# Kiteretsu77/This_and_That_VDM

Hardware: AMD Instinct MI355X
Metric: denoise-steps/sec (14-frame 256x448 VGL, 25 steps) (higher is better)
Workload: dtype bf16; 1 GPU; VGL denoise step: GestureNet ControlNet + spatio-temporal UNet + per-frame CFG + Euler, latent 14x4x32x56, CFG batch 2, 78 context tokens, heads (5,10,20,20); mode=vgl, requests_per_gpu=1, parallelism=1 independent request(s), one per GPU; RCCL weight broadcast at start-up only, hipgraph=True, finite_output=True, spatial_self_attention=bf16, weights_identical_on_all_ranks=True

## Files before the change

this_and_that_vdm_amd/csrc/gemm.hip:

```cpp
#include <stdlib.h>
#include "gemm_kernel.h"

namespace ttg {
void launch_bf16(GemmP& p, int cfg, hipStream_t st);
void launch_f16(GemmP& p, int cfg, hipStream_t st);
void launch_f32(GemmP& p, int cfg, hipStream_t st);
void launch_sq320_bf16(const GemmP& p, hipStream_t st);
void launch_sq320_f16(const GemmP& p, hipStream_t st);
void launch_pp_bf16(GemmP& p, hipStream_t st);
void launch_pp_f16(GemmP& p, hipStream_t st);
void launch_w320(GemmP& p, hipStream_t st, int bm, bool bf16);
}
using namespace ttg;

namespace {
inline int gemm_taps(int mode) { return mode == 1 || mode == 3 ? 9 : (mode == 2 ? 3 : 1); }

int env_int(const char* name, int dflt) { const char* e = getenv(name); return e ? atoi(e) : dflt; }
int big_tile_bits(int on) { return on == 0 ? 0 : (on == 2 ? 1 : (on == 3 ? 11 : (on == 4 ? 7 : 15))); }
struct Knobs {
  int forced_cfg = env_int("TT_GEMM_CFG", -1);
  int group_m = env_int("TT_GEMM_GROUP_M", 0);
  int forced_split = env_int("TT_GEMM_SPLITK", -1);
  int deep = env_int("TT_GEMM_DEEP", 1);
  int small64 = env_int("TT_GEMM_SMALL64", 2);
  int sq320 = env_int("TT_GEMM_SQ320", 2);
  int sq320_rowvec = env_int("TT_SQ320_ROWVEC", 1);
  int sq320_min_rows = env_int("TT_SQ320_MIN_ROWS", 131072);
  int pp = env_int("TT_GEMM_PP", 1);
  int pp_geglu_min_tiles = env_int("TT_PP_GEGLU_MIN_TILES", 400);
  int pp_geglu_min_fill = env_int("TT_PP_GEGLU_MIN_FILL", 75);
  int pp_min_tiles = env_int("TT_PP_MIN_TILES", 460);
  int pp_min_fill = env_int("TT_PP_MIN_FILL", 90);
  int pp_split_whole = env_int("TT_PP_SPLIT_WHOLE", 1);
  int w320 = big_tile_bits(env_int("TT_GEMM_W320", 1));
  int w320_force = env_int("TT_W320_FORCE", 0);
  int w320_min_fill = env_int("TT_W320_MIN_FILL", 60);
  int f32_split = env_int("TT_F32_SPLIT", 0) ? 1 : 0;
  int f32_split_min_tiles = env_int("TT_F32_SPLIT_MIN_TILES", 160);
// ... 109 lines not shown
    if (head.m < a->m && pp_ok(&head)) return head.m;
  }
  return 0;
}
void pp_split(const TtGemmArgs* a, int rows, TtGemmArgs* head, TtGemmArgs* tail) {
  const size_t es = 2;
  *head = *a; *tail = *a;
  head->m = rows;
  tail->m = a->m - rows;
  tail->a0 = (const char*)a->a0 + (size_t)rows * a->lda0 * es;
  tail->out = (char*)a->out + (size_t)rows * a->ldo * es;
}

const TileCfg& tile_of(int dtype, int cfg) { return dtype == TT_F32 ? kCfgsF32[cfg] : kCfgs[cfg]; }
bool ln_capable(int cfg) { return kCfgs[cfg].ln; }
bool mode3_capable(int cfg) { return kCfgs[cfg].m3; }
Plan mode3_plan(const TtGemmArgs* a, Plan pl) {
  if (a->mode != 3 || a->dtype == TT_F32 || knobs().forced_cfg >= 0 || mode3_capable(pl.cfg)) return pl;
  if (pl.cfg == 20) return Plan{16, pl.splitk};
  const long b128 = (long)ceil_div(a->m, 128) * ceil_div(a->n, 128), b12864 = (long)ceil_div(a->m, 128) * ceil_div(a->n, 64);
  return Plan{b128 >= 384 ? 11 : (b12864 >= 384 ? 1 : 2), 1};
}
bool mode3_served(const TtGemmArgs* a, const Plan& pl) { return a->mode != 3 || tile_of(a->dtype, pl.cfg).m3; }
Plan plan_for(const TtGemmArgs* a) {
  if (a->dtype == TT_F32) {
    const int split_min = knobs().f32_split_min_tiles;
    if (knobs().f32_split) {
      const long b128 = (long)ceil_div(a->m, 128) * ceil_div(a->n, 128);
      const long kt = (long)gemm_taps(a->mode) * (a->k0 + a->k1) / 32;
      if (knobs().f32_splitk && !a->geglu && !a->ln_fold && !a->out_col_hw && b128 < split_min && kt >= 64) {
        long sp = 448 / b128;
        if (sp > kt / 16) sp = kt / 16;
        if (sp > 16) sp = 16;
        if (sp >= 2) return Plan{0, (int)sp};
      }
    }
    return Plan{plan_f32(a->m, a->n, knobs().f32_split ? split_min : 256), 1};
  }
  const long ktot = (long)gemm_taps(a->mode) * (a->k0 + a->k1);
  const bool allow = !a->geglu && !a->ln_fold && !a->out_fp8;
  const bool k128 = (a->k0 & 127) == 0 && (a->k1 & 127) == 0;
  const bool wide_ok = !(a->residual || a->blend || a->rowvec);
  Plan pl = make_plan(knobs().forced_cfg, a->m, a->n, ktot, allow, wide_ok, a->mode == 0, k128);
  if (a->ln_fold && !ln_capable(pl.cfg))
    pl = make_plan(-1, a->m, a->n, ktot, false, wide_ok, a->mode == 0);
  return mode3_plan(a, pl);
}
// ... 14 lines not shown
  if (sq) return Route{Kind::SQ320, -1, 1, 0};
  if (big) return Route{big == 1 ? Kind::W320 : Kind::W320H, -1, 1, 0};
  if (const int split = w320_split(a)) return Route{Kind::W320H_SPLIT, -1, split, 0};
  return tiled_route(a, plan_for(a));
}
Route granted_route(const TtGemmArgs* a, Route r) {
  if (r.kind == Kind::W320H_SPLIT && !ws_fits(a, r.splitk)) r = tiled_route(a, plan_for(a));
  if (r.kind == Kind::TILED && r.splitk > 1 && (!ws_fits(a, r.splitk) || slab_bytes(a, r.splitk) >= ((size_t)1 << 31))) r = tiled_route(a, unsplit_plan(a));
  return r;
}
Route resolve(const TtGemmArgs* a) { return granted_route(a, wanted_route(a)); }

TileCfg route_tile(const TtGemmArgs* a, const Route& r) {
  switch (r.kind) {
    case Kind::PP: case Kind::PP_TWO_PART: return TileCfg{-1, 256, 256, 64, 0, 2, 4};
    case Kind::SQ320: return TileCfg{-1, SQ_ROWS, SQ_N, SQ_K, a->residual ? 3 : 5, 1, SQ_WAVES};
    case Kind::W320: return TileCfg{-1, 256, 320, 64, 0, 4, 2};
    case Kind::W320H: case Kind::W320H_SPLIT: return TileCfg{-1, 128, 320, 64, 0, 2, 2};
    default: return tile_of(a->dtype, r.cfg);
  }
}

int32_t stats_rows_on(const TtGemmArgs* a, const Route& r) {
  if (a->geglu || a->out_fp8 || a->out_f32 || a->out_col_hw > 0 || a->ln_fold == 2) return 0;
  if (r.kind == Kind::PP || r.kind == Kind::PP_TWO_PART || r.kind == Kind::SQ320 || r.kind == Kind::UNSUPPORTED) return 0;
  const int seg = a->stats_seg;
  if (r.splitk != 1) {
    if (seg <= 0) return 0;
    for (int rows = seg < 128 ? seg : 128; rows > 0; --rows)
      if (seg % rows == 0) return a->m % rows == 0 ? rows : 0;
    return 0;
  }
  const TileCfg t = route_tile(a, r);
  if (a->blend && !(a->blend == a->residual && a->ld_blend == a->ld_res)) return 0;
  if (a->rowvec && a->rowvec_rows < 32 && !(a->rowvec_rows == 1 && a->rowvec_mod == 2)) return 0;
  if (t.bm > 128 && t.bn != 320 && a->residual) return 0;
  if (a->dtype == TT_F32 && knobs().f32_split && a->residual) return 0;
  if (t.bn == 320 || t.nst == 0) {
    if (a->m % t.bm) return 0;
    return (t.bm == 128 && seg > 0 && seg % 128 && seg % 64 == 0) ? 64 : t.bm;
  }
  const int wave_rows = t.bm / t.wgm;
  const int rows = (seg <= 0 || seg % t.bm == 0) ? t.bm : (seg % wave_rows == 0 ? wave_rows : t.bm);
  return a->m % rows == 0 ? rows : 0;
}
int32_t gn_fused_on(const TtGemmArgs* a, const Route& r) {
  if (a->dtype == TT_F32 || a->geglu || a->out_fp8 || a->out_f32 || a->out_col_hw > 0 || a->stats_out) return 0;
  const int seg = a->stats_seg;
  if (seg <= 0 || a->m % seg || (a->n & 127)) return 0;
  if (r.kind != Kind::W320H_SPLIT && r.kind != Kind::TILED) return 0;
  if (r.splitk <= 1) return 0;
  return splitk_gn_rows(seg, a->n, nullptr) > 0 ? 1 : 0;
}
}

int tt_internal_f32_split() { return knobs().f32_split; }

extern "C" int tt_gemm_set_tile_override(int32_t cfg) {
  if (cfg < -1 || cfg >= kNumCfgs) TT_FAIL(TT_EINVAL, "tt_gemm_set_tile_override: cfg %d (valid -1..%d)", cfg, kNumCfgs - 1);
  knobs().forced_cfg = cfg;
  return TT_OK;
}
extern "C" int tt_gemm_set_streaming_square(int32_t on) {
  knobs().sq320 = on == 2 ? 2 : (on ? 1 : 0);
  return TT_OK;
}
extern "C" int tt_gemm_set_f32_split(int32_t on) { knobs().f32_split = on ? 1 : 0; return TT_OK; }
extern "C" int tt_gemm_set_big_tile(int32_t on) { knobs().w320 = big_tile_bits(on); return TT_OK; }

extern "C" int tt_gemm_plan(const TtGemmArgs* a, int32_t cfg[7]) {
  if (!a || !cfg || a->m <= 0 || a->n <= 0) TT_FAIL(TT_EINVAL, "tt_gemm_plan: bad arguments");
  const Route r = resolve(a);
  if (r.kind == Kind::UNSUPPORTED)
    TT_FAIL(TT_EUNSUPPORTED, "tt_gemm_plan: forced tile configuration %d has no mode-3 variant (mode 3 is built for 1, 2, 11, 16)", r.cfg);
  const TileCfg t = route_tile(a, r);
  cfg[0] = t.bm; cfg[1] = t.bn; cfg[2] = t.bk; cfg[3] = t.nst; cfg[4] = t.wgm; cfg[5] = t.wgn; cfg[6] = r.splitk;
  return TT_OK;
}

extern "C" int32_t tt_gemm_stats_rows(const TtGemmArgs* a) {
  if (!a || a->m <= 0 || a->n <= 0) return 0;
  return stats_rows_on(a, resolve(a));
}

extern "C" int32_t tt_gemm_gn_fused(const TtGemmArgs* a) {
  if (!a || a->m <= 0 || a->n <= 0) return 0;
  return gn_fused_on(a, resolve(a));
}

extern "C" size_t tt_gemm_ws_bytes(const TtGemmArgs* a) {
  if (!a || a->m <= 0 || a->n <= 0) return 0;
  const Route r = wanted_route(a);
  if (r.kind == Kind::PP_TWO_PART) { TtGemmArgs head, tail; pp_split(a, r.head_rows, &head, &tail); return tt_gemm_ws_bytes(&tail); }
  return (r.kind == Kind::W320H_SPLIT || r.kind == Kind::TILED) && r.splitk > 1 ? slab_bytes(a, r.splitk) : 0;
// ... 28 lines not shown
  p.blend = (const char*)a->blend; p.ld_blend = a->ld_blend; p.alpha = a->alpha;
  const int es = a->dtype == TT_F32 ? 4 : 2;
  p.out = (char*)a->out; p.ldo = a->ldo; p.out_f32 = a->dtype == TT_F32 ? 0 : a->out_f32;
  p.out_col_hw = a->out_col_hw; p.out_col_hwp = a->out_col_hwp;
  p.ln_fold = a->ln_fold; p.ln_eps = a->ln_eps; p.out_fp8 = a->out_fp8; p.stats = a->stats_out; p.stat_rows = a->gn_out ? a->stats_seg : (a->stats_out ? stats_rows_on(a, r) : 0);
  p.f32_split = a->dtype == TT_F32 ? knobs().f32_split : 0;
  p.presplit = a->presplit;
  if (a->presplit) {
    if ((a->presplit & ~3) || a->dtype != TT_F32 || !p.f32_split)
      TT_FAIL(TT_EINVAL, "tt_gemm: presplit operands need TT_F32 with tt_gemm_set_f32_split(1)");
    if (((a->presplit & 1) && a->ln_fold == 1) || ((a->presplit & 2) && a->ln_fold == 2))
      TT_FAIL(TT_EINVAL, "tt_gemm: the LayerNorm statistics cannot be taken from a pre-split operand");
    if ((a->presplit & 1) && a->mode != 0) TT_FAIL(TT_EINVAL, "tt_gemm: a pre-split A operand is a Linear operand (mode 0)");
  }
  p.gn_out = (char*)a->gn_out; p.ld_gn = a->ld_gn; p.gn_gamma = a->gn_gamma; p.gn_beta = a->gn_beta; p.gn_eps = a->gn_eps; p.gn_silu = a->gn_silu;
  if (p.mode == 1 || p.mode == 3) {
    if (p.nimg <= 0 || p.hin <= 0 || p.win <= 0 || p.hout <= 0 || p.wout <= 0 || p.stride < 1)
      TT_FAIL(TT_EINVAL, "tt_gemm: conv geometry");
    if ((long)p.nimg * p.hout * p.wout != p.m) TT_FAIL(TT_EINVAL, "tt_gemm: m != nimg*hout*wout");
  }
  if (p.mode == 2) {
    if (p.frames <= 0 || p.hw <= 0 || p.m % ((long)p.frames * p.hw)) TT_FAIL(TT_EINVAL, "tt_gemm: tconv geometry");
  }
  p.taps = gemm_taps(p.mode);
  {
    const long rows = p.mode == 1 || p.mode == 3 ? (long)p.nimg * p.hin * p.win : (long)p.m;
    const long a0b = ((rows - 1) * p.lda0 + p.k0) * es, a1b = p.k1 ? ((rows - 1) * p.lda1 + p.k1) * es : 16;
    const long wb = ((long)(p.n - 1) * p.ldw + (long)p.taps * (p.k0 + p.k1)) * es;
    if (a0b >= (1L << 31) || a1b >= (1L << 31) || wb >= (1L << 31))
      TT_FAIL(TT_EUNSUPPORTED, "tt_gemm: operand larger than 2 GiB (32-bit buffer offsets)");
    p.a0_bytes = (unsigned)a0b; p.a1_bytes = (unsigned)a1b; p.w_bytes = (unsigned)wb;
    const long n_out = p.geglu ? p.n / 2 : p.n;
    const long outb = ((long)(p.m - 1) * p.ldo + (p.out_col_hw > 0 ? p.ldo : n_out)) * (p.out_f32 ? 4 : (p.out_fp8 ? 1 : es));
    const long resb = p.residual ? ((long)(p.m - 1) * p.ld_res + p.n) * es : 0;
    const long blb = p.blend ? ((long)(p.m - 1) * p.ld_blend + p.n) * es : 0;
    long rv_last = p.rowvec ? (p.m - 1) / p.rowvec_rows : 0;
    if (p.rowvec_mod > 0 && rv_last > p.rowvec_mod - 1) rv_last = p.rowvec_mod - 1;
    const long rvb = p.rowvec ? (rv_last * p.ld_rowvec + p.n) * 4 : 0;
    if (outb >= (1L << 31) || resb >= (1L << 31) || blb >= (1L << 31) || rvb >= (1L << 31))
      TT_FAIL(TT_EUNSUPPORTED, "tt_gemm: epilogue operand larger than 2 GiB (32-bit buffer offsets)");
    p.out_bytes = (unsigned)outb; p.res_bytes = (unsigned)resb; p.blend_bytes = (unsigned)blb;
    p.bias_bytes = p.bias ? (unsigned)p.n * 4u : 0u; p.rowvec_bytes = (unsigned)rvb;
  }
  p.splitk = r.splitk; p.group_m = 1;
  p.group_m_override = r.kind == Kind::PP || r.kind == Kind::TILED ? knobs().group_m : 0;
  p.ws = r.splitk > 1 ? (float*)a->ws : nullptr;
  p.ws_bytes = r.splitk > 1 ? (unsigned)slab_bytes(a, r.splitk) : 0u;
  return TT_OK;
}
}

extern "C" int tt_gemm(const TtGemmArgs* a, tt_stream_t stream) {
  if (!a || !a->a0 || !a->w || !a->out) TT_FAIL(TT_EINVAL, "tt_gemm: null operand");
  if (a->m <= 0 || a->n <= 0 || a->k0 <= 0) TT_FAIL(TT_EINVAL, "tt_gemm: empty problem m=%d n=%d k0=%d", a->m, a->n, a->k0);
  if (a->dtype != TT_BF16 && a->dtype != TT_F16 && a->dtype != TT_F32) TT_FAIL(TT_EINVAL, "tt_gemm: bad dtype");
  if ((a->k0 & 7) || (a->k1 & 7) || (a->n & 3)) TT_FAIL(TT_EINVAL, "tt_gemm: k0/k1 must be multiples of 8 and n of 4");
  if ((a->lda0 & 7) || (a->k1 && (a->lda1 & 7)) || (a->ldw & 7)) TT_FAIL(TT_EINVAL, "tt_gemm: row strides must be multiples of 8 elements");
  if (a->k1 && !a->a1) TT_FAIL(TT_EINVAL, "tt_gemm: k1 > 0 without a1");
  if (a->mode < 0 || a->mode > 3) TT_FAIL(TT_EINVAL, "tt_gemm: bad mode %d", a->mode);
  if (a->mode == 3 && a->upsample) TT_FAIL(TT_EINVAL, "tt_gemm: mode 3 (bottom / right zero padding) has no fused upsample");
  const Route r = resolve(a);
  if (r.kind == Kind::PP_TWO_PART) {
    TtGemmArgs head, tail;
    pp_split(a, r.head_rows, &head, &tail);
    const int rc = tt_gemm(&head, stream);
    return rc != TT_OK ? rc : tt_gemm(&tail, stream);
  }
  GemmP p;
  if (const int rc = fill_params(a, r, p)) return rc;
  hipStream_t st = (hipStream_t)stream;
  const bool bf16 = a->dtype == TT_BF16;
  switch (r.kind) {
    case Kind::PP: if (bf16) launch_pp_bf16(p, st); else launch_pp_f16(p, st); break;
    case Kind::SQ320: if (bf16) launch_sq320_bf16(p, st); else launch_sq320_f16(p, st); break;
    case Kind::W320: launch_w320(p, st, 256, bf16); break;
    case Kind::W320H: case Kind::W320H_SPLIT: launch_w320(p, st, 128, bf16); break;
    case Kind::TILED:
      if (bf16) launch_bf16(p, r.cfg, st);
      else if (a->dtype == TT_F16) launch_f16(p, r.cfg, st);
      else launch_f32(p, r.cfg, st);
      break;
    default:
      TT_FAIL(TT_EUNSUPPORTED, "tt_gemm: forced tile configuration %d has no mode-3 variant (mode 3 is built for 1, 2, 11, 16)", r.cfg);
// ... 5 lines not shown
```

this_and_that_vdm_amd/csrc/gemm_kernel.h:

```cpp
#pragma once
#include <stdlib.h>
#include <type_traits>
#include "common.h"

namespace ttg {


struct FastDiv { unsigned mul, sh; };
static inline FastDiv make_fastdiv(long d_) {
  unsigned long long d = d_ < 1 ? 1 : (unsigned long long)d_;
  unsigned l = 0;
  while ((1ull << l) < d) ++l;
  FastDiv f;
  f.mul = (unsigned)(((1ull << (31 + l)) + d - 1) / d);
  f.sh = 31 + l;
  return f;
}
__device__ __forceinline__ int fdiv(int n, const FastDiv& f) { return (int)(((unsigned long long)(unsigned)n * f.mul) >> f.sh); }

struct GemmP {
  const char* a0; const char* a1;
  int k0, k1; long lda0, lda1;
  const char* w; long ldw;
  int m, n, mode;
  int nimg, hin, win, hout, wout, stride, upsample;
  int frames, hw;
  const float* bias; float acc_scale;
  const float* rowvec; int rowvec_rows; long ld_rowvec;
  int rowvec_mod;
  int geglu;
  const char* residual; long ld_res;
  const char* blend; long ld_blend; float alpha;
  char* out; long ldo; int out_f32;
  int out_col_hw, out_col_hwp;
  int nk0, nk1, taps, kt_total;
  int tiles_m, tiles_n;
  int group_m_override;
  int group_m;
  unsigned a0_bytes, a1_bytes, w_bytes;
  unsigned out_bytes, res_bytes, blend_bytes, bias_bytes, rowvec_bytes, ws_bytes;
  int splitk;
  float* ws;
  int ln_fold; float ln_eps;
  int out_fp8;
  float* stats;
  int stat_rows;
  char* gn_out; long ld_gn;
  const float* gn_gamma; const float* gn_beta; float gn_eps; int gn_silu;
  int f32_split;
  int presplit;
  FastDiv fd_splitk, fd_per_group, fd_group_m, fd_last_rows, fd_per_tap, fd_hwo, fd_wout, fd_hw, fd_frames, fd_rv_rows, fd_rv_mod;
};

__device__ __forceinline__ unsigned pack4_fp8(const float* v) {
  int w = 0;
  w = __builtin_amdgcn_cvt_pk_fp8_f32(__builtin_amdgcn_fmed3f(v[0], -448.f, 448.f), __builtin_amdgcn_fmed3f(v[1], -448.f, 448.f), w, false);
  w = __builtin_amdgcn_cvt_pk_fp8_f32(__builtin_amdgcn_fmed3f(v[2], -448.f, 448.f), __builtin_amdgcn_fmed3f(v[3], -448.f, 448.f), w, true);
  return (unsigned)w;
}
__device__ __forceinline__ void st32(__amdgpu_buffer_rsrc_t r, int off, unsigned a) {
  __builtin_amdgcn_raw_buffer_store_b32(a, r, off, 0, 0);
}

__device__ __forceinline__ void colstat_strip(const char* ebuf, int q_per_row, int lane, float* srow_sum, float* srow_sq, bool first) {
// ... 164 lines not shown
  static_assert(SPLIT || (!PRE_A && !PRE_B), "pre-split operands belong to the split variants");
  static_assert(!SPLIT || std::is_same<Tag, f32_tag>::value, "split products are a TT_F32 mode");
  constexpr bool PAD_BR = KMODE == 5;
  constexpr int MODE = PAD_BR ? 1 : (KMODE >= 3 ? 0 : KMODE);
  constexpr int LN = KMODE == 3 || KMODE == 4 ? KMODE - 2 : 0;
  TL(0);
  kernarg_touch<sizeof(GemmP)>();
  typedef typename Elem<Tag>::quad_t quad_t;
  constexpr int ES = Elem<Tag>::ES, EPC = Elem<Tag>::EPC;
  constexpr int NT = 64 * WGM * WGN;
  constexpr int CPR = BK / EPC;
  constexpr int WTM = BM / WGM, WTN = BN / WGN, FM = WTM / 32, FN = WTN / 32;
  constexpr int AR = (BM * CPR + NT - 1) / NT, BR = (BN * CPR + NT - 1) / NT;
  constexpr int A_BYTES = AR * NT * 16, B_BYTES = BR * NT * 16, STAGE = A_BYTES + B_BYTES;
  constexpr int G = AR + BR;
  constexpr int RPI = NT / CPR;
  static_assert(NT % CPR == 0 && NST >= 2 && NST <= 5 && WTM % 32 == 0 && WTN % 32 == 0, "tile/threads mismatch");

  const int tid = threadIdx.x, lane = tid & 63;
  const int wid = __builtin_amdgcn_readfirstlane(tid >> 6);

  int bid = xcd_remap(blockIdx.x, gridDim.x);
  int split = 0;
  if (p.splitk > 1) { const int t = fdiv(bid, p.fd_splitk); split = bid - t * p.splitk; bid = t; }
  int tile_m, tile_n;
  {
    const int gm = p.group_m;
    const int per_group = gm * p.tiles_n;
    const int grp = fdiv(bid, p.fd_per_group);
    const int first = grp * gm;
    const int r = bid - grp * per_group;
    const bool full = first + gm <= p.tiles_m;
    const int rows = full ? gm : p.tiles_m - first;
    tile_n = full ? fdiv(r, p.fd_group_m) : fdiv(r, p.fd_last_rows);
    tile_m = first + (r - tile_n * rows);
  }
  const int m0 = tile_m * BM, n0 = tile_n * BN;
  const int kt_lo = p.splitk > 1 ? fdiv(p.kt_total * split, p.fd_splitk) : 0;
  const int KT = p.splitk > 1 ? fdiv(p.kt_total * (split + 1), p.fd_splitk) - kt_lo : p.kt_total;

  constexpr int INV = (int)0x80000000;
  const __amdgpu_buffer_rsrc_t ra0 = __builtin_amdgcn_make_buffer_rsrc((void*)p.a0, 0, p.a0_bytes, 0x00020000);
  const __amdgpu_buffer_rsrc_t ra1 = __builtin_amdgcn_make_buffer_rsrc((void*)(p.a1 ? p.a1 : p.a0), 0, p.a1_bytes, 0x00020000);
  const __amdgpu_buffer_rsrc_t rw = __builtin_amdgcn_make_buffer_rsrc((void*)p.w, 0, p.w_bytes, 0x00020000);
  const int crow = tid / CPR, cchunk = tid % CPR;
  int a_chunk[AR];
  int va0[AR], va1[AR];
  int a_img[AR], a_y[AR], a_x[AR];
  bool a_valid[AR];
#pragma unroll
  for (int i = 0; i < AR; ++i) {
    const int r = i * RPI + crow;
    a_chunk[i] = cchunk ^ tile_swz<CPR>(r);
    const int gm = m0 + r;
    a_valid[i] = gm < p.m && r < BM;
    const int g = a_valid[i] ? gm : 0;
    va0[i] = va1[i] = INV;
    a_img[i] = a_y[i] = a_x[i] = 0;
    if constexpr (MODE == 0) {
      if (a_valid[i]) {
        va0[i] = (int)(((long)g * p.lda0 + a_chunk[i] * EPC) * ES);
        va1[i] = (int)(((long)g * p.lda1 + a_chunk[i] * EPC) * ES);
// ... 18 lines not shown
    const int gn = n0 + r;
    vb[i] = (gn < p.n && r < BN) ? (int)(((long)gn * p.ldw + b_chunk[i] * EPC) * ES) : INV;
  }

  int s_tap, s_src, s_kc;
  {
    const int per_tap = p.nk0 + p.nk1;
    s_tap = kt_lo ? fdiv(kt_lo, p.fd_per_tap) : 0;
    const int rem = kt_lo - s_tap * per_tap;
    s_src = rem >= p.nk0 ? 1 : 0;
    s_kc = rem - (s_src ? p.nk0 : 0);
  }
  bool tap_dirty = true;
  auto stage = [&](int slot) {
    if constexpr (MODE != 0) {
      if (tap_dirty) {
        tap_dirty = false;
#pragma unroll
        for (int i = 0; i < AR; ++i) {
          bool ok = a_valid[i];
          long row;
          if constexpr (MODE == 1) {
            constexpr int OFF = PAD_BR ? 0 : 1;
            const int dy = s_tap / 3 - OFF, dx = s_tap - (dy + OFF) * 3 - OFF;
            int iy = a_y[i] * p.stride + dy, ix = a_x[i] * p.stride + dx;
            const bool up = !PAD_BR && p.upsample;
            const int hv = up ? p.hin * 2 : p.hin, wv = up ? p.win * 2 : p.win;
            ok = ok && iy >= 0 && iy < hv && ix >= 0 && ix < wv;
            if (up) { iy >>= 1; ix >>= 1; }
            row = ((long)a_img[i] * p.hin + iy) * p.win + ix;
          } else {
            const int f = a_img[i] + s_tap - 1;
            ok = ok && f >= 0 && f < p.frames;
            row = (long)a_y[i] + (long)(s_tap - 1) * p.hw;
          }
          va0[i] = ok ? (int)((row * p.lda0 + a_chunk[i] * EPC) * ES) : INV;
          va1[i] = ok ? (int)((row * p.lda1 + a_chunk[i] * EPC) * ES) : INV;
        }
      }
    }
    const int src = __builtin_amdgcn_readfirstlane(s_src);
    const int ksrc = src ? p.k1 : p.k0;
    const int kbase = __builtin_amdgcn_readfirstlane(s_kc) * BK;
    const bool tail = kbase + BK > ksrc;
    char* lds_a = smem + slot * STAGE + wid * 1024;
    char* lds_b = smem + slot * STAGE + A_BYTES + wid * 1024;
    const int soff_a = kbase * ES;
// ... 372 lines not shown
      for (int j = 0; j < FN; ++j) cs[j * 32 + l31] = rs[j];
    }
  }
  const float* colscale = (const float*)(smem + CS_OFF + wid * 1024);

  TL(3);
  if (!direct) {
    const __amdgpu_buffer_rsrc_t r_bias = make_rsrc(p.bias, p.bias_bytes);
    const __amdgpu_buffer_rsrc_t r_out = p.splitk > 1 ? make_rsrc(p.ws, p.ws_bytes) : make_rsrc(p.out, p.out_bytes);
    auto strip_off = [](int row, int quad, int nq) { return row * 256 + ((quad ^ (row & (nq - 1))) << 4); };
    char* ebuf = smem + wid * 8192;
    static_assert(WGM * WGN * 8192 <= NST * STAGE, "epilogue strips do not fit the ring");
    if (!p.geglu) {
      float4 bias4[NCH];
#pragma unroll
      for (int c = 0; c < NCH; ++c) {
        const int q_per_row = ((2 * c + 1 < FN) ? 2 : 1) * 8;
        const int gn = n0 + wc * WTN + c * 64 + (lane % q_per_row) * 4;
        bias4[c] = ld128f(r_bias, gn < p.n ? gn * 4 : kInv);
      }
      const float alpha = p.blend ? p.alpha : 0.0f, one_m_alpha = 1.0f - alpha;
      __syncthreads();
      TL(4);
      auto run = [&](auto film_tag, auto inpass_tag, auto out8_tag, auto stats_tag) {
        constexpr bool FILM = decltype(film_tag)::value, INPASS = decltype(inpass_tag)::value, OUT8 = decltype(out8_tag)::value;
        constexpr bool STATS = decltype(stats_tag)::value;
        const __amdgpu_buffer_rsrc_t r_rv = make_rsrc(p.rowvec, (FILM || INPASS) ? p.rowvec_bytes : 0);
        const __amdgpu_buffer_rsrc_t r_bl = make_rsrc(p.blend, INPASS ? p.blend_bytes : 0);
        const __amdgpu_buffer_rsrc_t r_res = make_rsrc(p.residual, (INPASS && !EARLY_RES) ? p.res_bytes : 0);
        const int rv_rows = p.rowvec ? p.rowvec_rows : 1;
        const bool parity = FILM && p.rowvec_mod == 2 && rv_rows == 1;
        auto wrap = [&](int g) { return p.rowvec_mod > 0 ? g - fdiv(g, p.fd_rv_mod) * p.rowvec_mod : g; };
        float* sstage = (float*)(smem + STAT_OFF) + wid * (2 * WTN);
#pragma unroll
        for (int i = 0; i < FM; ++i) {
          const int mb = m0 + wr * WTM + i * 32;
          const int grp_raw = fdiv(mb, p.fd_rv_rows);
          const int grp0 = parity ? 0 : wrap(grp_raw), grp1 = parity ? 1 : wrap(grp_raw + 1);
          const int grp_split = parity ? mb : (grp_raw + 1) * rv_rows;
          const int sel_split = parity ? 0x7fffffff : grp_split, sel_odd = parity ? 1 : 0;
#pragma unroll
          for (int jc = 0; jc < FN; jc += 2) {
            const int nfr = (jc + 1 < FN) ? 2 : 1;
            const int q_per_row = nfr * 8;
            const int rows_per_pass = 64 / q_per_row;
            const int qq = lane % q_per_row, rr = lane / q_per_row;
            const int gn = n0 + wc * WTN + jc * 32 + qq * 4;
            const float4 b4 = bias4[jc / 2];
// ... 22 lines not shown
              for (int k = 0; k < PB; ++k) {
                const int pass = pb + k;
                rqv[k] = blv[k] = zero_quad<Tag>();
                rvv[k] = make_float4(0.f, 0.f, 0.f, 0.f);
                if (pass * rows_per_pass < 32) {
                  const int gm = mb + pass * rows_per_pass + rr;
                  const bool ok = gm < p.m && gn < p.n;
                  if constexpr (EARLY_RES) rqv[k] = resv[i][jc / 2][pass];
                  else if constexpr (INPASS) rqv[k] = ldq<Tag>(r_res, ok ? (int)(((long)gm * p.ld_res + gn) * ES) : kInv);
                  if constexpr (INPASS) {
                    rvv[k] = ld128f(r_rv, ok ? (int)(((long)wrap(fdiv(gm, p.fd_rv_rows)) * p.ld_rowvec + gn) * 4) : kInv);
                    blv[k] = ldq<Tag>(r_bl, ok ? (int)(((long)gm * p.ld_blend + gn) * ES) : kInv);
                  }
                }
              }
#pragma unroll
              for (int k = 0; k < PB; ++k) {
                const int pass = pb + k;
                if (pass * rows_per_pass < 32) {
                  const int r = pass * rows_per_pass + rr;
                  const float4 t = *(const float4*)(ebuf + strip_off(r, qq, q_per_row));
                  const int gm = mb + r;
                  const bool ok = gm < p.m && gn < p.n;
                  if (p.splitk > 1) {
                    st128f(r_out, ok ? (int)((((long)split * p.m + gm) * p.n + gn) * 4) : kInv, t);
                  } else {
                    float v[4] = {(t.x * cs4.x + b4.x) * p.acc_scale, (t.y * cs4.y + b4.y) * p.acc_scale,
                                  (t.z * cs4.z + b4.z) * p.acc_scale, (t.w * cs4.w + b4.w) * p.acc_scale};
                    const quad_t rq = rqv[k];
                    quad_t bq = rq;
                    if constexpr (FILM) {
                      const float4 f = ((gm >= sel_split) | ((gm & sel_odd) != 0)) ? film_hi : film_lo;
                      v[0] += f.x; v[1] += f.y; v[2] += f.z; v[3] += f.w;
                    }
                    if constexpr (INPASS) {
                      v[0] += rvv[k].x; v[1] += rvv[k].y; v[2] += rvv[k].z; v[3] += rvv[k].w;
                      bq = (p.blend && !blend_is_res) ? blv[k] : rq;
                    }
                    float r4[4], b4v[4];
                    quad_to_f32<Tag>(rq, r4);
                    quad_to_f32<Tag>(bq, b4v);
#pragma unroll
                    for (int e = 0; e < 4; ++e) v[e] = alpha * b4v[e] + one_m_alpha * (v[e] + r4[e]);
                    if constexpr (OUT8) st32(r_out, ok ? (int)((long)gm * p.ldo + gn) : kInv, pack4_fp8(v));
                    else {
                      const quad_t packed = f32_to_quad<Tag>(v);
                      if constexpr (ES == 2) st64(r_out, ok ? (int)(((long)gm * p.ldo + gn) * ES) : kInv, packed.x, packed.y);
                      else stq<Tag>(r_out, ok ? (int)(((long)gm * p.ldo + gn) * ES) : kInv, v);
                      if constexpr (STATS) {
                        float sv[4];
                        quad_to_f32<Tag>(packed, sv);
                        const bool live = gm < p.m;
                        *(float4*)(ebuf + strip_off(r, qq, q_per_row)) = make_float4(live ? sv[0] : 0.f, live ? sv[1] : 0.f, live ? sv[2] : 0.f, live ? sv[3] : 0.f);
                      }
                    }
                  }
                }
              }
            }
            if constexpr (STATS) colstat_strip(ebuf, q_per_row, lane, sstage + jc * 32, sstage + WTN + jc * 32, i == 0);
          }
        }
      };
      const bool inpass = (p.blend && !blend_is_res) || (p.rowvec && p.rowvec_rows < 32 && !(p.rowvec_mod == 2 && p.rowvec_rows == 1)) ||
                          (!EARLY_RES && p.residual);
      constexpr std::false_type no{};
      constexpr std::true_type yes{};
      const bool kstats = p.stats && p.splitk == 1;
      if (inpass) run(no, yes, no, no);
      else if (p.rowvec) { if (kstats) run(yes, no, no, yes); else run(yes, no, no, no); }
      else if (MODE == 0 && ES == 2 && p.out_fp8) {
        if constexpr (MODE == 0 && ES == 2) run(no, no, yes, no);
      } else { if (kstats) run(no, no, no, yes); else run(no, no, no, no); }
      if (kstats) {
        __syncthreads();
        const float* st0 = (const float*)(smem + STAT_OFF);
        if (p.stat_rows == BM) {
          for (int c = tid; c < BN; c += NT) {
            const int wcc = c / WTN, col = c - wcc * WTN;
            float a = 0.f, b = 0.f;
#pragma unroll
            for (int w = 0; w < WGM; ++w) {
              const float* row = st0 + (w * WGN + wcc) * (2 * WTN);
              a += row[col]; b += row[WTN + col];
            }
            if (n0 + c < p.n) {
              p.stats[((long)tile_m * 2) * p.n + n0 + c] = a;
              p.stats[((long)tile_m * 2 + 1) * p.n + n0 + c] = b;
            }
          }
        } else {
          for (int c = tid; c < BN * WGM; c += NT) {
            const int w = c / BN, cc = c - w * BN, wcc = cc / WTN, col = cc - wcc * WTN;
            const float* row = st0 + (w * WGN + wcc) * (2 * WTN);
            const long srow = (long)tile_m * WGM + w;
            if (n0 + cc < p.n && srow * WTM < p.m) {
// ... 380 lines not shown
    else if (mr == 4) hipLaunchKernelGGL((splitk_epilogue_gn_kernel<Tag, 4>), grid, block, 0, st, p, rl_n);
    else hipLaunchKernelGGL((splitk_epilogue_gn_kernel<Tag, 8>), grid, block, 0, st, p, rl_n);
    return;
  }
  if (p.stats) {
    hipLaunchKernelGGL(splitk_epilogue_stats_kernel<Tag>, dim3(p.m / p.stat_rows, (p.n + 31) / 32), dim3(256), 0, st, p);
    return;
  }
  long blocks = ((long)p.m * (p.n >> 2) + 255) / 256;
  if (blocks > 2048) blocks = 2048;
  hipLaunchKernelGGL(splitk_epilogue_kernel<Tag>, dim3((unsigned)blocks), dim3(256), 0, st, p);
}

template <typename Tag, int BM, int BN, int BK, int NST, int WGM, int WGN, int MODE>
void launch_mode(const GemmP& p, hipStream_t st) {
  constexpr int NT_ = 64 * WGM * WGN, CPR_ = BK / Elem<Tag>::EPC;
  constexpr size_t lds = (size_t)NST * (((BM * CPR_ + NT_ - 1) / NT_) + ((BN * CPR_ + NT_ - 1) / NT_)) * NT_ * 16
                         + ((MODE & 7) == 4 ? WGM * WGN * 1024 : 0);
  static_assert(lds + (size_t)WGM * WGN * 2 * (BN / WGN) * sizeof(float) <= 160 * 1024, "LDS ring (+ the statistics staging rows) exceeds 160 KiB");
  static_assert((MODE & 7) != 4 || BN / WGN <= 256, "column-scale array: 1 KiB per wave");
  constexpr size_t stat_lds = (size_t)WGM * WGN * 2 * (BN / WGN) * sizeof(float);
  static unsigned long long attr_done = 0;
  tt_lds_opt_in((const void*)gemm_kernel<Tag, BM, BN, BK, NST, WGM, WGN, MODE>, (int)(lds + stat_lds), &attr_done);
  hipLaunchKernelGGL((gemm_kernel<Tag, BM, BN, BK, NST, WGM, WGN, MODE>), dim3(p.tiles_m * p.tiles_n * p.splitk),
                     dim3(64 * WGM * WGN), (p.stats && p.splitk == 1) ? lds + stat_lds : lds, st, p);
  if (p.splitk > 1) launch_splitk_epilogue<Tag>(p, st);
}

static inline void fill_fastdivs(GemmP& p) {
  p.fd_splitk = make_fastdiv(p.splitk);
  p.fd_per_group = make_fastdiv((long)p.group_m * p.tiles_n);
  p.fd_group_m = make_fastdiv(p.group_m);
  p.fd_last_rows = make_fastdiv(p.tiles_m % p.group_m ? p.tiles_m % p.group_m : p.group_m);
  p.fd_per_tap = make_fastdiv(p.nk0 + p.nk1);
  p.fd_hwo = make_fastdiv((long)p.hout * p.wout);
  p.fd_wout = make_fastdiv(p.wout);
  p.fd_hw = make_fastdiv(p.hw);
  p.fd_frames = make_fastdiv(p.frames);
  p.fd_rv_rows = make_fastdiv(p.rowvec ? p.rowvec_rows : 1);
  p.fd_rv_mod = make_fastdiv(p.rowvec_mod > 0 ? p.rowvec_mod : 1);
}

template <typename Tag, int BM, int BN, int BK, int NST, int WGM, int WGN, bool LNOK = false, bool M3OK = false>
void launch_cfg(GemmP& p, hipStream_t st) {
  p.tiles_m = ceil_div(p.m, BM);
  p.tiles_n = ceil_div(p.n, BN);
  {
    constexpr int NT_ = 64 * WGM * WGN, CPR_ = BK / Elem<Tag>::EPC;
    constexpr long lds_ = (long)NST * (((BM * CPR_ + NT_ - 1) / NT_) + ((BN * CPR_ + NT_ - 1) / NT_)) * NT_ * 16;
    const int window = 32 * (lds_ * 2 <= 160 * 1024 ? 2 : 1);
    int gm = p.group_m_override;
    if (gm <= 0) {
      gm = 1;
      if (p.tiles_n > 8)
        while (gm * 2 * BM * gm * 2 <= (long)window * BN && gm * 2 <= p.tiles_m) gm *= 2;
    }
    p.group_m = gm < 1 ? 1 : (gm > p.tiles_m ? p.tiles_m : gm);
  }
  p.nk0 = ceil_div(p.k0, BK); p.nk1 = p.k1 ? ceil_div(p.k1, BK) : 0;
  p.kt_total = p.taps * (p.nk0 + p.nk1);
  fill_fastdivs(p);
  if (p.mode == 3) {
    if constexpr (M3OK) {
      if constexpr (std::is_same<Tag, f32_tag>::value) {
        if (p.f32_split) {
          if (p.presplit & 2) launch_mode<Tag, BM, BN, BK, NST, WGM, WGN, 13 + 16>(p, st); else launch_mode<Tag, BM, BN, BK, NST, WGM, WGN, 13>(p, st);
          return;
        }
      }
      launch_mode<Tag, BM, BN, BK, NST, WGM, WGN, 5>(p, st);
    }
    return;
  }
  if constexpr (std::is_same<Tag, f32_tag>::value) {
    if (p.f32_split) {
      const int pre = p.presplit & 3;
      if (LNOK && p.ln_fold == 1) {
        if (pre & 2) launch_mode<Tag, BM, BN, BK, NST, WGM, WGN, 11 + 16>(p, st); else launch_mode<Tag, BM, BN, BK, NST, WGM, WGN, 11>(p, st);
        return;
      }
      if (LNOK && p.ln_fold == 2) {
        if (pre & 1) launch_mode<Tag, BM, BN, BK, NST, WGM, WGN, 12 + 32>(p, st); else launch_mode<Tag, BM, BN, BK, NST, WGM, WGN, 12>(p, st);
        return;
// ... 82 lines not shown
```

this_and_that_vdm_amd/ops.py:

```python
from __future__ import annotations

import ctypes as C
import os
from typing import Optional, Tuple

import torch

from . import _lib
from ._lib import TT_BF16, TT_F16, TT_F32, TtAttnArgs, TtConvArgs, TtEncAttnArgs, TtGemmArgs, check
from .packing import PreSplitF32


PROFILE = None


def _prof_begin():
    if PROFILE is None:
        return None
    e = torch.cuda.Event(enable_timing=True)
    e.record()
    return e


def _prof_end(start, name, flops, shape=None):
# ... 150 lines not shown
    sbuf = gnbuf = None
    if stats and gn is not None and GN_FUSED:
        g.stats_seg = int(stats)
        if lib.tt_gemm_gn_fused(C.byref(g)):
            gnbuf = torch.empty((g.m, n), dtype=out.dtype, device=a0.device)
            g.gn_out, g.ld_gn, g.gn_gamma, g.gn_beta, g.gn_eps, g.gn_silu = gnbuf.data_ptr(), n, _p(gn[0]), _p(gn[1]), float(gn[2]), int(bool(gn[3]))
    if stats and gnbuf is None and GN_TILES and g.m * n <= GN_TILES_MAX_ELEMS:
        g.stats_seg = int(stats) if GN_TILES_SEG else 0
        srows = lib.tt_gemm_stats_rows(C.byref(g))
        if srows > 0 and lib.tt_groupnorm_tiles_supported(int(stats), n, srows, g.dtype):
            sbuf = torch.empty(((g.m + srows - 1) // srows, 2, n), dtype=torch.float32, device=a0.device)
            g.stats_out = sbuf.data_ptr()
    ev = _prof_begin()
    check(lib.tt_gemm(C.byref(g), _stream()), "tt_gemm")
    serial = _wrote(out)
    if sbuf is not None:
        out._tt_stats = (sbuf, srows, serial, out.data_ptr(), tuple(out.shape))
    if gnbuf is not None:
        out._tt_gn = (gnbuf, gn[0].data_ptr(), gn[1].data_ptr(), float(gn[2]), bool(gn[3]), int(stats), serial, out.data_ptr(), tuple(out.shape))
    if ev is not None:
        cfg = (C.c_int32 * 7)()
        lib.tt_gemm_plan(C.byref(g), cfg)
        taps = 9 if mode in (1, 3) else (3 if mode == 2 else 1)
        tag = _TAG[g.dtype]
        if cfg[3] == 0 and cfg[1] == 320:
            kname = f"gemm_w320{'h' if cfg[0] == 128 else ''}_kernel<{tag}, {mode}, {int(bool(ln_fold))}>"
        elif cfg[3] == 0:
            kname = f"gemm_pp_kernel<{tag}, {int(bool(ln_fold))}, {int(bool(geglu))}>"
        elif cfg[0] == 32 and cfg[1] == 320:
            kname = f"sq320_kernel<{tag}, {'true' if residual is not None else 'false'}>"
        else:
            kmode = (5 if mode == 3 else mode if not ln_fold else 2 + ln_fold) + (8 if (g.dtype == TT_F32 and _F32_SPLIT) else 0)
            if mode == 3:
                kmode += 16 if g.presplit & 2 else 0
            kname = f"gemm_kernel<{tag}, {', '.join(str(v) for v in cfg[:6])}, {kmode}>"
        _prof_end(ev, kname, 2.0 * g.m * n * taps * (g.k0 + g.k1),
                  shape=(mode, g.m, n, taps * (g.k0 + g.k1), int(geglu), int(residual is not None)))
    return out


CONV3X3_FUSED = os.environ.get("TT_CONV3X3", "0") == "1"


def conv3x3_supported(h: int, w: int, c0: int, c1: int, n: int, dtype: torch.dtype) -> bool:
    if dtype not in (torch.bfloat16, torch.float16):
        return False
# ... 564 lines not shown
```

this_and_that_vdm_amd/packing.py:

```python
from __future__ import annotations

import os

import torch


def pack_conv3x3(w: torch.Tensor) -> torch.Tensor:
    o, i = w.shape[:2]
    return w.permute(0, 2, 3, 1).reshape(o, 9 * i).contiguous()


def pack_tconv3(w: torch.Tensor) -> torch.Tensor:
    o, i = w.shape[:2]
    return w[:, :, :, 0, 0].permute(0, 2, 1).reshape(o, 3 * i).contiguous()


def pack_conv1x1(w: torch.Tensor) -> torch.Tensor:
    return w.reshape(w.shape[0], w.shape[1]).contiguous()


def pack_geglu(w: torch.Tensor, b: torch.Tensor):
    n2, k = w.shape
    half = n2 // 2
    assert half % 8 == 0
    wp = w.view(2, half // 8, 8, k).permute(1, 0, 2, 3).reshape(n2, k).contiguous()
    bp = b.view(2, half // 8, 8).permute(1, 0, 2).reshape(n2).contiguous()
    return wp, bp


def pad_rows(w: torch.Tensor, multiple: int) -> torch.Tensor:
    n = w.shape[0]
    np_ = (n + multiple - 1) // multiple * multiple
# ... 98 lines not shown
```

this_and_that_vdm_amd/svd/layers.py:

```python
from __future__ import annotations

import math
import os
from dataclasses import dataclass
from typing import Dict, List, Optional, Tuple

import torch
import torch.nn as nn

from .. import ops
from ..packing import fold_layernorm, pack_conv1x1, pack_conv3x3, pack_geglu, pack_tconv3, permute_q_rows, zero_sum_round


ZERO_CTX_TEMPORAL = os.environ.get("TT_ZERO_CTX_T", "1") != "0"
ATTN_V_ROWS = os.environ.get("TT_ATTN_V_ROWS", "1") != "0"
MERGE_FRAMES = os.environ.get("TT_XATTN_MERGE_FRAMES", "1") != "0"


@dataclass
class Geom:
    batch: int
    frames: int
    h: int
    w: int
    batch0: int = 0
    batch_total: int = 0
    requests: int = 1

    @property
    def n(self):
        return self.batch * self.frames

    @property
    def hw(self):
        return self.h * self.w

    @property
    def m(self):
        return self.n * self.hw
# ... 296 lines not shown
        super().__init__()
        if not use_conv or padding != 1:
            raise NotImplementedError("SVD uses Downsample2D(use_conv=True, padding=1)")
        self.conv = nn.Conv2d(channels, out_channels or channels, 3, stride=2, padding=1)

    def pack(self, reg, dtype):
        self.w, self.b = pack_conv3x3(self.conv.weight.detach().to(dtype)), _f32(self.conv.bias)

    def forward(self, x, g: Geom):
        ho, wo = (g.h + 2 - 3) // 2 + 1, (g.w + 2 - 3) // 2 + 1
        out = ops.gemm(x, self.w, mode=1, conv=(g.n, g.h, g.w, ho, wo, 2, 0), bias=self.b, stats=ho * wo)
        return out, Geom(g.batch, g.frames, ho, wo, g.batch0, g.batch_total, g.requests)


class Upsample2D(_Packable):
    def __init__(self, channels: int, use_conv: bool = False, use_conv_transpose: bool = False,
                 out_channels: Optional[int] = None, name: str = "conv"):
        super().__init__()
        if not use_conv or use_conv_transpose:
            raise NotImplementedError("SVD uses Upsample2D(use_conv=True)")
        self.conv = nn.Conv2d(channels, out_channels or channels, 3, padding=1)

    def pack(self, reg, dtype):
        self.w, self.b = pack_conv3x3(self.conv.weight.detach().to(dtype)), _f32(self.conv.bias)

    def forward(self, x, g: Geom):
        out = ops.gemm(x, self.w, mode=1, conv=(g.n, g.h, g.w, 2 * g.h, 2 * g.w, 1, 1), bias=self.b, stats=4 * g.hw)
        return out, Geom(g.batch, g.frames, 2 * g.h, 2 * g.w, g.batch0, g.batch_total, g.requests)


class Attention(nn.Module):

    def __init__(self, query_dim: int, cross_attention_dim: Optional[int] = None, heads: int = 8, dim_head: int = 64,
                 dropout: float = 0.0, bias: bool = False, out_bias: bool = True):
        super().__init__()
        self.inner_dim, self.heads, self.dim_head = heads * dim_head, heads, dim_head
        self.is_cross = cross_attention_dim is not None
        cross = cross_attention_dim if self.is_cross else query_dim
        self.to_q = nn.Linear(query_dim, self.inner_dim, bias=bias)
        self.to_k = nn.Linear(cross, self.inner_dim, bias=bias)
        self.to_v = nn.Linear(cross, self.inner_dim, bias=bias)
        self.to_out = nn.ModuleList([nn.Linear(self.inner_dim, query_dim, bias=out_bias), nn.Dropout(dropout)])
        if dim_head not in (64, 128):
            raise NotImplementedError(f"attention head_dim {dim_head}: kernels are built for 64 and 128")


class GEGLU(nn.Module):
    def __init__(self, dim_in: int, dim_out: int):
        super().__init__()
        self.proj = nn.Linear(dim_in, dim_out * 2)
# ... 259 lines not shown
```

Measured before the change: 35.74 denoise-steps/s.

## Decompose nearest-upsample + 3x3 conv into four 2x2 sub-pixel phase convolutions

Upsample2D's nearest-2x followed by 3x3 conv is rewritten as four phase-specific 2x2 convolutions over the low-resolution input. Weights are pre-summed per phase at pack time, and the tiled GEMM kernel runs four slices that pick taps and scatter output rows by phase. This cuts the tap count from 9 per output pixel to 4, removing redundant MACs on the duplicated pixels. In exchange the fused GroupNorm stats output is dropped for these convs, so downstream norms must compute stats separately, and the pre-summed weights change rounding slightly.

```diff
diff --git a/this_and_that_vdm_amd/csrc/gemm.hip b/this_and_that_vdm_amd/csrc/gemm.hip
--- a/this_and_that_vdm_amd/csrc/gemm.hip
+++ b/this_and_that_vdm_amd/csrc/gemm.hip
@@ -15,6 +15,16 @@
 
 namespace {
 inline int gemm_taps(int mode) { return mode == 1 || mode == 3 ? 9 : (mode == 2 ? 3 : 1); }
+
+inline bool is_up2(const TtGemmArgs* a) { return a->mode == 1 && a->upsample == 2; }
+const char* up2_refusal(const TtGemmArgs* a) {
+  if (a->stride != 1 || a->hout != 2 * a->hin || a->wout != 2 * a->win) return "stride 1 with hout = 2 hin and wout = 2 win";
+  if (a->a1 || a->k1) return "one source (no a1 / k1)";
+  if (a->residual || a->blend || a->rowvec) return "a bias-only epilogue (no residual / blend / rowvec)";
+  if (a->stats_out || a->gn_out) return "no stats_out / gn_out";
+  if (a->geglu || a->ln_fold || a->out_fp8 || a->out_f32 || a->out_col_hw) return "no geglu / ln_fold / out_fp8 / out_f32 / out_col_hw";
+  return nullptr;
+}
 
 int env_int(const char* name, int dflt) { const char* e = getenv(name); return e ? atoi(e) : dflt; }
 int big_tile_bits(int on) { return on == 0 ? 0 : (on == 2 ? 1 : (on == 3 ? 11 : (on == 4 ? 7 : 15))); }
@@ -170,7 +180,15 @@
   return Plan{b128 >= 384 ? 11 : (b12864 >= 384 ? 1 : 2), 1};
 }
 bool mode3_served(const TtGemmArgs* a, const Plan& pl) { return a->mode != 3 || tile_of(a->dtype, pl.cfg).m3; }
+Plan up2_plan(const TtGemmArgs* a) {
+  const long blocks = 4L * ceil_div(a->m / 4, 128) * ceil_div(a->n, 128);
+  if (a->dtype == TT_F32) return Plan{blocks >= 256 ? 0 : 1, 1};
+  const int f = knobs().forced_cfg;
+  if (f >= 0 && f < kNumCfgs) return Plan{f, 1};
+  return Plan{blocks > 256 ? 11 : 16, 1};
+}
 Plan plan_for(const TtGemmArgs* a) {
+  if (is_up2(a)) return up2_plan(a);
   if (a->dtype == TT_F32) {
     const int split_min = knobs().f32_split_min_tiles;
     if (knobs().f32_split) {
@@ -231,6 +249,7 @@
 }
 
 int32_t stats_rows_on(const TtGemmArgs* a, const Route& r) {
+  if (is_up2(a)) return 0;
   if (a->geglu || a->out_fp8 || a->out_f32 || a->out_col_hw > 0 || a->ln_fold == 2) return 0;
   if (r.kind == Kind::PP || r.kind == Kind::PP_TWO_PART || r.kind == Kind::SQ320 || r.kind == Kind::UNSUPPORTED) return 0;
   const int seg = a->stats_seg;
@@ -254,6 +273,7 @@
   return a->m % rows == 0 ? rows : 0;
 }
 int32_t gn_fused_on(const TtGemmArgs* a, const Route& r) {
+  if (is_up2(a)) return 0;
   if (a->dtype == TT_F32 || a->geglu || a->out_fp8 || a->out_f32 || a->out_col_hw > 0 || a->stats_out) return 0;
   const int seg = a->stats_seg;
   if (seg <= 0 || a->m % seg || (a->n & 127)) return 0;
@@ -279,6 +299,7 @@
 
 extern "C" int tt_gemm_plan(const TtGemmArgs* a, int32_t cfg[7]) {
   if (!a || !cfg || a->m <= 0 || a->n <= 0) TT_FAIL(TT_EINVAL, "tt_gemm_plan: bad arguments");
+  if (is_up2(a)) if (const char* why = up2_refusal(a)) TT_FAIL(TT_EINVAL, "tt_gemm_plan: upsample = 2 needs %s", why);
   const Route r = resolve(a);
   if (r.kind == Kind::UNSUPPORTED)
     TT_FAIL(TT_EUNSUPPORTED, "tt_gemm_plan: forced tile configuration %d has no mode-3 variant (mode 3 is built for 1, 2, 11, 16)", r.cfg);
@@ -353,7 +374,7 @@
   if (p.mode == 2) {
     if (p.frames <= 0 || p.hw <= 0 || p.m % ((long)p.frames * p.hw)) TT_FAIL(TT_EINVAL, "tt_gemm: tconv geometry");
   }
-  p.taps = gemm_taps(p.mode);
+  p.taps = is_up2(a) ? 16 : gemm_taps(p.mode);
   {
     const long rows = p.mode == 1 || p.mode == 3 ? (long)p.nimg * p.hin * p.win : (long)p.m;
     const long a0b = ((rows - 1) * p.lda0 + p.k0) * es, a1b = p.k1 ? ((rows - 1) * p.lda1 + p.k1) * es : 16;
@@ -377,6 +398,12 @@
   p.group_m_override = r.kind == Kind::PP || r.kind == Kind::TILED ? knobs().group_m : 0;
   p.ws = r.splitk > 1 ? (float*)a->ws : nullptr;
   p.ws_bytes = r.splitk > 1 ? (unsigned)slab_bytes(a, r.splitk) : 0u;
+  p.slices = r.splitk; p.phases = 0;
+  if (is_up2(a)) {
+    if (r.kind != Kind::TILED || r.splitk != 1) TT_FAIL(TT_EUNSUPPORTED, "tt_gemm: upsample = 2 runs on the tiled template, unsplit");
+    p.phases = 1; p.upsample = 0;
+    p.m = p.nimg * p.hin * p.win; p.hout = p.hin; p.wout = p.win;
+  }
   return TT_OK;
 }
 }
@@ -390,6 +417,7 @@
   if (a->k1 && !a->a1) TT_FAIL(TT_EINVAL, "tt_gemm: k1 > 0 without a1");
   if (a->mode < 0 || a->mode > 3) TT_FAIL(TT_EINVAL, "tt_gemm: bad mode %d", a->mode);
   if (a->mode == 3 && a->upsample) TT_FAIL(TT_EINVAL, "tt_gemm: mode 3 (bottom / right zero padding) has no fused upsample");
+  if (is_up2(a)) if (const char* why = up2_refusal(a)) TT_FAIL(TT_EINVAL, "tt_gemm: upsample = 2 needs %s", why);
   const Route r = resolve(a);
   if (r.kind == Kind::PP_TWO_PART) {
     TtGemmArgs head, tail;
diff --git a/this_and_that_vdm_amd/csrc/gemm_kernel.h b/this_and_that_vdm_amd/csrc/gemm_kernel.h
--- a/this_and_that_vdm_amd/csrc/gemm_kernel.h
+++ b/this_and_that_vdm_amd/csrc/gemm_kernel.h
@@ -40,6 +40,8 @@
   unsigned a0_bytes, a1_bytes, w_bytes;
   unsigned out_bytes, res_bytes, blend_bytes, bias_bytes, rowvec_bytes, ws_bytes;
   int splitk;
+  int slices;
+  int phases;
   float* ws;
   int ln_fold; float ln_eps;
   int out_fp8;
@@ -250,7 +252,7 @@
 
   int bid = xcd_remap(blockIdx.x, gridDim.x);
   int split = 0;
-  if (p.splitk > 1) { const int t = fdiv(bid, p.fd_splitk); split = bid - t * p.splitk; bid = t; }
+  if (p.slices > 1) { const int t = fdiv(bid, p.fd_splitk); split = bid - t * p.slices; bid = t; }
   int tile_m, tile_n;
   {
     const int gm = p.group_m;
@@ -264,8 +266,8 @@
     tile_m = first + (r - tile_n * rows);
   }
   const int m0 = tile_m * BM, n0 = tile_n * BN;
-  const int kt_lo = p.splitk > 1 ? fdiv(p.kt_total * split, p.fd_splitk) : 0;
-  const int KT = p.splitk > 1 ? fdiv(p.kt_total * (split + 1), p.fd_splitk) - kt_lo : p.kt_total;
+  const int kt_lo = p.slices > 1 ? fdiv(p.kt_total * split, p.fd_splitk) : 0;
+  const int KT = p.slices > 1 ? fdiv(p.kt_total * (split + 1), p.fd_splitk) - kt_lo : p.kt_total;
 
   constexpr int INV = (int)0x80000000;
   const __amdgpu_buffer_rsrc_t ra0 = __builtin_amdgcn_make_buffer_rsrc((void*)p.a0, 0, p.a0_bytes, 0x00020000);
@@ -330,7 +332,8 @@
           long row;
           if constexpr (MODE == 1) {
             constexpr int OFF = PAD_BR ? 0 : 1;
-            const int dy = s_tap / 3 - OFF, dx = s_tap - (dy + OFF) * 3 - OFF;
+            int dy = s_tap / 3 - OFF, dx = s_tap - (dy + OFF) * 3 - OFF;
+            if (!PAD_BR && p.phases) { dy = ((s_tap >> 1) & 1) - 1 + (split >> 1); dx = (s_tap & 1) - 1 + (split & 1); }
             int iy = a_y[i] * p.stride + dy, ix = a_x[i] * p.stride + dx;
             const bool up = !PAD_BR && p.upsample;
             const int hv = up ? p.hin * 2 : p.hin, wv = up ? p.win * 2 : p.win;
@@ -749,8 +752,10 @@
       const float alpha = p.blend ? p.alpha : 0.0f, one_m_alpha = 1.0f - alpha;
       __syncthreads();
       TL(4);
-      auto run = [&](auto film_tag, auto inpass_tag, auto out8_tag, auto stats_tag) {
+      auto run = [&](auto film_tag, auto inpass_tag, auto out8_tag, auto stats_tag, auto phase_tag) {
         constexpr bool FILM = decltype(film_tag)::value, INPASS = decltype(inpass_tag)::value, OUT8 = decltype(out8_tag)::value;
+        constexpr bool PHASE = decltype(phase_tag)::value;
+        const int ph_row0 = (split >> 1) * 2 * p.win + (split & 1), ph_hw = p.hin * p.win;
         constexpr bool STATS = decltype(stats_tag)::value;
         const __amdgpu_buffer_rsrc_t r_rv = make_rsrc(p.rowvec, (FILM || INPASS) ? p.rowvec_bytes : 0);
         const __amdgpu_buffer_rsrc_t r_bl = make_rsrc(p.blend, INPASS ? p.blend_bytes : 0);
@@ -819,6 +824,11 @@
                   const float4 t = *(const float4*)(ebuf + strip_off(r, qq, q_per_row));
                   const int gm = mb + r;
                   const bool ok = gm < p.m && gn < p.n;
+                  int orow = gm;
+                  if constexpr (PHASE) {
+                    const int img = fdiv(gm, p.fd_hwo), rem = gm - img * ph_hw, y = fdiv(rem, p.fd_wout), x = rem - y * p.win;
+                    orow = (img * p.hin + y) * 4 * p.win + 2 * x + ph_row0;
+                  }
                   if (p.splitk > 1) {
                     st128f(r_out, ok ? (int)((((long)split * p.m + gm) * p.n + gn) * 4) : kInv, t);
                   } else {
@@ -842,8 +852,8 @@
                     if constexpr (OUT8) st32(r_out, ok ? (int)((long)gm * p.ldo + gn) : kInv, pack4_fp8(v));
                     else {
                       const quad_t packed = f32_to_quad<Tag>(v);
-                      if constexpr (ES == 2) st64(r_out, ok ? (int)(((long)gm * p.ldo + gn) * ES) : kInv, packed.x, packed.y);
-                      else stq<Tag>(r_out, ok ? (int)(((long)gm * p.ldo + gn) * ES) : kInv, v);
+                      if constexpr (ES == 2) st64(r_out, ok ? (int)(((long)orow * p.ldo + gn) * ES) : kInv, packed.x, packed.y);
+                      else stq<Tag>(r_out, ok ? (int)(((long)orow * p.ldo + gn) * ES) : kInv, v);
                       if constexpr (STATS) {
                         float sv[4];
                         quad_to_f32<Tag>(packed, sv);
@@ -864,11 +874,13 @@
       constexpr std::false_type no{};
       constexpr std::true_type yes{};
       const bool kstats = p.stats && p.splitk == 1;
-      if (inpass) run(no, yes, no, no);
-      else if (p.rowvec) { if (kstats) run(yes, no, no, yes); else run(yes, no, no, no); }
+      if (inpass) run(no, yes, no, no, no);
+      else if (p.rowvec) { if (kstats) run(yes, no, no, yes, no); else run(yes, no, no, no, no); }
       else if (MODE == 0 && ES == 2 && p.out_fp8) {
-        if constexpr (MODE == 0 && ES == 2) run(no, no, yes, no);
-      } else { if (kstats) run(no, no, no, yes); else run(no, no, no, no); }
+        if constexpr (MODE == 0 && ES == 2) run(no, no, yes, no, no);
+      } else if (MODE == 1 && !PAD_BR && p.phases) {
+        if constexpr (MODE == 1 && !PAD_BR) run(no, no, no, no, yes);
+      } else { if (kstats) run(no, no, no, yes, no); else run(no, no, no, no, no); }
       if (kstats) {
         __syncthreads();
         const float* st0 = (const float*)(smem + STAT_OFF);
@@ -1295,13 +1307,13 @@
   constexpr size_t stat_lds = (size_t)WGM * WGN * 2 * (BN / WGN) * sizeof(float);
   static unsigned long long attr_done = 0;
   tt_lds_opt_in((const void*)gemm_kernel<Tag, BM, BN, BK, NST, WGM, WGN, MODE>, (int)(lds + stat_lds), &attr_done);
-  hipLaunchKernelGGL((gemm_kernel<Tag, BM, BN, BK, NST, WGM, WGN, MODE>), dim3(p.tiles_m * p.tiles_n * p.splitk),
+  hipLaunchKernelGGL((gemm_kernel<Tag, BM, BN, BK, NST, WGM, WGN, MODE>), dim3(p.tiles_m * p.tiles_n * p.slices),
                      dim3(64 * WGM * WGN), (p.stats && p.splitk == 1) ? lds + stat_lds : lds, st, p);
   if (p.splitk > 1) launch_splitk_epilogue<Tag>(p, st);
 }
 
 static inline void fill_fastdivs(GemmP& p) {
-  p.fd_splitk = make_fastdiv(p.splitk);
+  p.fd_splitk = make_fastdiv(p.slices);
   p.fd_per_group = make_fastdiv((long)p.group_m * p.tiles_n);
   p.fd_group_m = make_fastdiv(p.group_m);
   p.fd_last_rows = make_fastdiv(p.tiles_m % p.group_m ? p.tiles_m % p.group_m : p.group_m);
@@ -1332,6 +1344,7 @@
   }
   p.nk0 = ceil_div(p.k0, BK); p.nk1 = p.k1 ? ceil_div(p.k1, BK) : 0;
   p.kt_total = p.taps * (p.nk0 + p.nk1);
+  p.slices = p.phases ? 4 : p.splitk;
   fill_fastdivs(p);
   if (p.mode == 3) {
     if constexpr (M3OK) {
diff --git a/this_and_that_vdm_amd/ops.py b/this_and_that_vdm_amd/ops.py
--- a/this_and_that_vdm_amd/ops.py
+++ b/this_and_that_vdm_amd/ops.py
@@ -196,6 +196,8 @@
         cfg = (C.c_int32 * 7)()
         lib.tt_gemm_plan(C.byref(g), cfg)
         taps = 9 if mode in (1, 3) else (3 if mode == 2 else 1)
+        if mode == 1 and g.upsample == 2:
+            taps = 4
         tag = _TAG[g.dtype]
         if cfg[3] == 0 and cfg[1] == 320:
             kname = f"gemm_w320{'h' if cfg[0] == 128 else ''}_kernel<{tag}, {mode}, {int(bool(ln_fold))}>"
diff --git a/this_and_that_vdm_amd/packing.py b/this_and_that_vdm_amd/packing.py
--- a/this_and_that_vdm_amd/packing.py
+++ b/this_and_that_vdm_amd/packing.py
@@ -8,6 +8,22 @@
 def pack_conv3x3(w: torch.Tensor) -> torch.Tensor:
     o, i = w.shape[:2]
     return w.permute(0, 2, 3, 1).reshape(o, 9 * i).contiguous()
+
+
+def pack_upsample_phases(w: torch.Tensor, dtype: torch.dtype) -> torch.Tensor:
+    o, i = w.shape[:2]
+    acc = torch.float64 if dtype == torch.float64 else torch.float32
+    ws = w.detach().to(dtype).to(acc)
+    rows = {0: ((0,), (1, 2)), 1: ((0, 1), (2,))}
+    out = torch.zeros((o, 2, 2, 2, 2, i), dtype=acc, device=w.device)
+    for py in (0, 1):
+        for px in (0, 1):
+            for r in (0, 1):
+                for c in (0, 1):
+                    for ky in rows[py][r]:
+                        for kx in rows[px][c]:
+                            out[:, py, px, r, c] += ws[:, :, ky, kx]
+    return out.reshape(o, 16 * i).to(dtype).contiguous()
 
 
 def pack_tconv3(w: torch.Tensor) -> torch.Tensor:
diff --git a/this_and_that_vdm_amd/svd/layers.py b/this_and_that_vdm_amd/svd/layers.py
--- a/this_and_that_vdm_amd/svd/layers.py
+++ b/this_and_that_vdm_amd/svd/layers.py
@@ -9,12 +9,13 @@
 import torch.nn as nn
 
 from .. import ops
-from ..packing import fold_layernorm, pack_conv1x1, pack_conv3x3, pack_geglu, pack_tconv3, permute_q_rows, zero_sum_round
+from ..packing import fold_layernorm, pack_conv1x1, pack_conv3x3, pack_geglu, pack_tconv3, pack_upsample_phases, permute_q_rows, zero_sum_round
 
 
 ZERO_CTX_TEMPORAL = os.environ.get("TT_ZERO_CTX_T", "1") != "0"
 ATTN_V_ROWS = os.environ.get("TT_ATTN_V_ROWS", "1") != "0"
 MERGE_FRAMES = os.environ.get("TT_XATTN_MERGE_FRAMES", "1") != "0"
+UPSAMPLE_PHASES = os.environ.get("TT_UPSAMPLE_PHASES", "1") != "0"
 
 
 @dataclass
@@ -357,10 +358,15 @@
         self.conv = nn.Conv2d(channels, out_channels or channels, 3, padding=1)
 
     def pack(self, reg, dtype):
-        self.w, self.b = pack_conv3x3(self.conv.weight.detach().to(dtype)), _f32(self.conv.bias)
+        self.phases = UPSAMPLE_PHASES
+        self.w = pack_upsample_phases(self.conv.weight, dtype) if self.phases else pack_conv3x3(self.conv.weight.detach().to(dtype))
+        self.b = _f32(self.conv.bias)
 
     def forward(self, x, g: Geom):
-        out = ops.gemm(x, self.w, mode=1, conv=(g.n, g.h, g.w, 2 * g.h, 2 * g.w, 1, 1), bias=self.b, stats=4 * g.hw)
+        if self.phases:
+            out = ops.gemm(x, self.w, mode=1, conv=(g.n, g.h, g.w, 2 * g.h, 2 * g.w, 1, 2), bias=self.b)
+        else:
+            out = ops.gemm(x, self.w, mode=1, conv=(g.n, g.h, g.w, 2 * g.h, 2 * g.w, 1, 1), bias=self.b, stats=4 * g.hw)
         return out, Geom(g.batch, g.frames, 2 * g.h, 2 * g.w, g.batch0, g.batch_total, g.requests)
 
 
```

Result: faster. 36.21 denoise-steps/s (median of 6 runs) (+1.3%).
